# juanaldayparejo/archnemesis-dist

Measured on AMD Instinct MI355X. Metric: forward-models/sec (10k nu x 100 layers), higher is better.
Workload: dtype f64; 1 GPU; synthetic correlated-k nadir thermal-emission forward model: 10000 wavenumbers x 100 layers x 8 gases, G=20, k-table 20Px15T (BASELINE configs[1], SURVEY C2); parallelism=replicas x1 (independent forward models)

## Files before the change

### archnemesis_dist_amd/csrc/ansfm_api.hip

```cpp
#include "ansfm_table_kernels.hip.h"
#include "ansfm_rt_params.h"
#include "ansfm_ctx.hip.h"

using namespace ansfm;

extern "C" {

int ansfm_abi_version(void) { return ANSFM_ABI_VERSION; }

int ansfm_create(int device, ansfm_ctx **out)
{
    if (!out) return ANSFM_ERR_INVALID;
    *out = nullptr;
    int ndev = 0;
    if (hipGetDeviceCount(&ndev) != hipSuccess || ndev <= 0 || device < 0 || device >= ndev)
        return ANSFM_ERR_HIP;
    ansfm_ctx *ctx = new ansfm_ctx();
    ctx->device = device;
    if (hipSetDevice(device) != hipSuccess) { delete ctx; return ANSFM_ERR_HIP; }
    if (hipStreamCreateWithFlags(&ctx->own_stream, hipStreamNonBlocking) != hipSuccess) {
        delete ctx;
        return ANSFM_ERR_HIP;
    }
    ctx->stream = ctx->own_stream;
// ... 95 lines not shown
        hipLaunchKernelGGL(k_table_check, dim3(nblk((size_t)W * Q, 256)), dim3(256), 0, ctx->stream, K_dev, W, G, Q,
                           ctx->d_flag.as<int>());
        hipLaunchKernelGGL(k_table_relayout, dim3((unsigned)(Wpad / kWave), nblk((size_t)Q, 64), (unsigned)G), dim3(256), 0,
                           ctx->stream, K_dev, ctx->lnK.as<double>(), W, Wpad, G, Q);
    }
    HIPCHK(hipGetLastError());
    int flag = 0;
    HIPCHK(hipMemcpyAsync(&flag, ctx->d_flag.p, sizeof(int), hipMemcpyDeviceToHost, ctx->stream));
    HIPCHK(hipStreamSynchronize(ctx->stream));
    ctx->W = W; ctx->Wpad = Wpad; ctx->G = G; ctx->NP = NP; ctx->NT = NT; ctx->S = S;
    ctx->monotone = (flag & 1) ? 0 : 1;
    ctx->has_boxed = (flag & 2) ? 1 : 0;
    ctx->h_delg.assign(DELG, DELG + G);
    ctx->h_wave.assign(WAVE, WAVE + W); ctx->h_press.assign(PRESS, PRESS + NP); ctx->h_temp.assign(TEMP, TEMP + NT);
    ctx->have_table = true;
    ctx->is_lbl = 0; ctx->temp2d = 0;
    ctx->lblrt = 0; ctx->st_n = 0;
    clear_continuum_sources(ctx);
    return build_table_gfast(ctx, Wpad, G, NP * NT * S, false);
}

int ansfm_upload_ktable(ansfm_ctx *ctx, int W, int G, int NP, int NT, int S, const double *K,
                        const double *PRESS, const double *TEMP, const double *WAVE, const double *DELG)
{
    CHECK_CTX(ctx);
    if (W <= 0 || G <= 0 || NP <= 0 || NT <= 0 || S <= 0 || !K) FAIL(ANSFM_ERR_INVALID, "upload_ktable: bad dims");
    HIPCHK(hipSetDevice(ctx->device));
    const size_t n = (size_t)W * G * NP * NT * S;
    HIPCHK(ctx->tmp_in.reserve(n * sizeof(double)));
    HIPCHK(hipMemcpyAsync(ctx->tmp_in.p, K, n * sizeof(double), hipMemcpyHostToDevice, ctx->stream));
// ... 183 lines not shown
        HIPCHK(hipMemcpyAsync(ctx->tmp_in.p, block.data(), block.size() * sizeof(float), hipMemcpyHostToDevice, ctx->stream));
        hipLaunchKernelGGL(k_kta_relayout, dim3(nblk(per_wave * Wpad, 256)), dim3(256), 0, ctx->stream, ctx->tmp_in.as<float>(),
                           ctx->lnK.as<double>(), W, Wpad, G, NP, NT, S, s, ctx->d_flag.as<int>());
        HIPCHK(hipGetLastError());
        HIPCHK(hipStreamSynchronize(ctx->stream));
    }
    int flag = 0;
    HIPCHK(hipMemcpyAsync(&flag, ctx->d_flag.p, sizeof(int), hipMemcpyDeviceToHost, ctx->stream));
    HIPCHK(hipStreamSynchronize(ctx->stream));
    ctx->tmp_in.release();
    ctx->W = W; ctx->Wpad = Wpad; ctx->G = G; ctx->NP = NP; ctx->NT = NT; ctx->S = S;
    ctx->monotone = (flag & 1) ? 0 : 1;
    ctx->has_boxed = (flag & 2) ? 1 : 0;
    ctx->h_delg = DELG; ctx->h_wave = WAVE; ctx->h_press = PRESS; ctx->h_temp = TEMP;
    ctx->have_table = true;
    ctx->is_lbl = lta ? 1 : 0; ctx->temp2d = (lta && hl.temp2d) ? 1 : 0;
    ctx->lblrt = 0; ctx->st_n = 0;
    clear_continuum_sources(ctx);
    if (lta) ctx->monotone = 1;
    ctx->grid_f32 = 1; ctx->delg_f32 = lta ? 0 : 1;
    return build_table_gfast(ctx, Wpad, G, NP * NT * S, lta);
}

int ansfm_upload_ktable_files(ansfm_ctx *ctx, int S, const char *const *paths, double wavemin, double wavemax)
{
    return upload_table_files(ctx, S, paths, wavemin, wavemax, false);
}

int ansfm_upload_lbltable_files(ansfm_ctx *ctx, int S, const char *const *paths, double wavemin, double wavemax)
{
// ... 60 lines not shown
}

int ansfm_last_merge_rowmajor(const ansfm_ctx *cctx, int64_t *merges, int64_t *merges_total)
{
    ansfm_ctx *ctx = const_cast<ansfm_ctx *>(cctx);
    CHECK_CTX(ctx);
    if (!merges || !merges_total) FAIL(ANSFM_ERR_INVALID, "last_merge_rowmajor: null argument");
    *merges = *merges_total = 0;
    if (ctx->d_flag.bytes < kFlagInts * sizeof(int)) return ANSFM_OK;
    HIPCHK(hipSetDevice(ctx->device));
    unsigned long long v[2] = {0, 0};
    HIPCHK(hipMemcpyAsync(v, ctx->d_flag.as<int>() + kFlagTileCounter + 8, sizeof v, hipMemcpyDeviceToHost, ctx->stream));
    HIPCHK(hipStreamSynchronize(ctx->stream));
    *merges = (int64_t)v[0];
    *merges_total = (int64_t)v[1];
    return ANSFM_OK;
}

static void launch_w_to_last(hipStream_t st, unsigned n_batch, const double *src, double *dst, int W, int Wpad, int X1, int X2,
                             int swap12, double padval, size_t src_stride = 0, size_t dst_stride = 0)
{
    const int X = X1 * X2;
    dim3 grid((unsigned)(Wpad / 32), (unsigned)((X + 31) / 32), n_batch);
    hipLaunchKernelGGL(k_transpose_w_last, grid, dim3(32, 8), 0, st, src, dst, W, Wpad, X1, X2, swap12, padval, src_stride,
                       dst_stride);
}

static int read_unsorted(ansfm_ctx *ctx, int *flag)
{
    *flag = 0;
// ... 1099 lines not shown
```

### archnemesis_dist_amd/csrc/ansfm_ctx.hip.h

```cpp
#pragma once
#include <hip/hip_runtime.h>
#include <stdio.h>
#include <stdlib.h>
#include <string.h>

#include <algorithm>
#include <cmath>
#include <initializer_list>
#include <memory>
#include <string>
#include <map>
#include <vector>

#pragma GCC visibility push(default)
#include "../../include/ansfm.h"
#pragma GCC visibility pop
#include "ansfm_merge_plan.h"

namespace ansfm {

struct DevBuf {
    void *p = nullptr;
    size_t bytes = 0;
    DevBuf() = default;
// ... 27 lines not shown

struct FusedRoute {
    DevBuf ws;
    size_t scratch_bytes = 0;
    int recorded = 0;
    hipEvent_t ev[3] = {nullptr, nullptr, nullptr};
    double ms[2] = {0.0, 0.0};
};

}

using ansfm::DevBuf;
using ansfm::FusedRoute;
using ansfm::LblrtIso;

constexpr int kFlagInts = 32, kFlagTileCounter = 16;

struct ansfm_ctx {
    int device = 0;
    hipStream_t own_stream = nullptr;
    hipStream_t stream = nullptr;
    std::string err;
    int num_cus = 256;

    int W = 0, Wpad = 0, G = 0, NP = 0, NT = 0, S = 0;
    int monotone = 0;
    int has_boxed = 1;
    std::vector<double> h_wave, h_press, h_temp;
    DevBuf dcont_gas;
    int dcont_gas_L = 0;
    unsigned grad_gas_mask = 0xFFFFFFFFu;
    std::map<const void *, size_t> merge_lds_allowed;
    ansfm::MergePlan last_merge;
    int merge_keys = 64;
    bool have_table = false;
    int grid_f32 = 0, delg_f32 = 0;
    int is_lbl = 0, temp2d = 0;
    DevBuf lnK, d_press, d_temp, d_wave, d_delg, d_flag;
    DevBuf lnKg;
    size_t lnKg_bytes = 0;
    std::vector<double> h_delg;
    DevBuf cia_tab, cia_idx, cia_lay, dust_kext;
    int cia_on = 0, cia_ispace = 0, cia_NWC = 0, cia_NPAIR = 0, cia_NPE = 0, cia_NT = 0, cia_nfrac = 0, cia_NPARA = 0, cia_NVMR = 0,
        cia_ico2 = -1, cia_in2 = -1, cia_ih2 = -1, cia_covers = 0;
    int dust_n = 0;

    DevBuf li, tau, scratch, cont_t, tmp_in, tmp_out, misc;
    DevBuf dspec_ref, map_out, map_b, map_batch;
    DevBuf dd_slot, dd_work, dd_in;
// ... 156 lines not shown
```

### archnemesis_dist_amd/csrc/ansfm_merge64.hip.h

```cpp
#pragma once
#include <hip/hip_runtime.h>
#include <stdint.h>
#include "ansfm_merge_common.hip.h"

namespace ansfm {

constexpr unsigned kLdsDG = 0, kLdsGORD = kMaxG * 8, kLdsDGF = (2 * kMaxG + 2) * 8, kLdsA = kLdsDGF + kMaxG * 4;


constexpr unsigned kLdsWT = kLdsA;
static_assert(kLdsA == kMergeLdsTables, "the plan's LDS arithmetic");
typedef double dbl2 __attribute__((ext_vector_type(2)));
constexpr unsigned kRecRow = 64u * 16u, kRecBin = 2u * kRecRow;

struct MergeElem {
    double ai, bc, bn, w;
    int ci, np;
};

struct MergeOrient {
    unsigned rbase, cbase;
    unsigned rsh, csh;
    unsigned inc;
};
// ... 249 lines not shown
    }
}
template <int NR>
__device__ __forceinline__ void merge_init(double (&R)[NR], int G, const MergeOrient &mo, double huge)
{
    const double c0 = lds_ld(mo.cbase);
#pragma unroll
    for (int i = 0; i < NR; ++i) {
        const unsigned long long b = (unsigned long long)__double_as_longlong(lds_ld(mo.rbase + (unsigned)(i < G ? i : 0) * 512u) + c0);
        R[i] = (i < G) ? __longlong_as_double((long long)((b & ~0x7FFULL) | (unsigned long long)((unsigned)i << mo.rsh))) : huge;
    }
    merge_init_order<NR>(R, G, huge);
}

template <int NR>
__device__ __forceinline__ bool merge_rowmajor_test(const double (&R)[NR], int G, const MergeOrient &mo)
{
    const double cl = lds_ld(mo.cbase + (unsigned)(G - 1) * 512u);
    const unsigned lowc = (unsigned)(G - 1) << mo.csh;
    bool fail = false;
#pragma unroll
    for (int i = 0; i + 1 < NR; ++i) {
        const unsigned long long b = (unsigned long long)__double_as_longlong(lds_ld(mo.rbase + (unsigned)(i < G ? i : 0) * 512u) + cl);
        const double last = __longlong_as_double((long long)((b & ~0x7FFULL) | (unsigned long long)(((unsigned)i << mo.rsh) | lowc)));
        fail |= (i + 1 < G) & !(last < R[i + 1]);
    }
    return __builtin_amdgcn_ballot_w64(fail) == 0;
}
__host__ __device__ constexpr int merge_rowmajor_sure_cols(int NR)
{
    return NR == 10 ? 9 : NR == 16 ? 11 : NR == 20 ? 17 : NR == 32 ? 21 : 2;
}
template <int NR>
__device__ __forceinline__ void merge_rowmajor_row(double ai, const double (&c)[NR], const double (&w)[NR], int G, WalkState &ws,
                                                   double *rec)
{
#pragma unroll
    for (int j = 0; j < NR; ++j) {
        if (j < merge_rowmajor_sure_cols(NR) || j < G) {
            MergeElem e;
            e.ai = ai; e.bc = c[j]; e.w = w[j];
// ... 64 lines not shown
```

### archnemesis_dist_amd/csrc/ansfm_merge_common.hip.h

```cpp
#pragma once
#include <hip/hip_runtime.h>
#include <stdint.h>
#include "ansfm_merge_plan.h"

namespace ansfm {

__device__ __forceinline__ double encode_lnk(double k)
{
    if (k > 0.0) return log(k);
    unsigned long long b = (unsigned long long)__double_as_longlong(k);
    unsigned long long box = 0x7FF8000000000000ULL | (b >> 13);
    return __longlong_as_double((long long)box);
}
__device__ __forceinline__ bool lnk_is_boxed(double x) { return x != x; }
__device__ __forceinline__ double lnk_unbox(double x)
{
    unsigned long long b = (unsigned long long)__double_as_longlong(x);
    return __longlong_as_double((long long)((b & 0x0007FFFFFFFFFFFFULL) << 13));
}

struct LayerInterp {
    int ipl, iph, itl, ith;
    double v, u, dudt;
};
// ... 45 lines not shown

struct OverlapParams {
    const double *lnK;
    const double *kin;
    const LayerInterp *li;
    const double *amount;
    const double *del_g;
    double *tau;
    double *scratch;
    int *err_flag;
    unsigned int *tile_counter;
    int W, Wpad, G, NT, S, L, n_models;
    int delg_f32;
    double g_ord[kMaxG + 2];
    const double *lnKg;
};
__host__ __device__ constexpr int gfast_stride(int G) { return (G + 1) & ~1; }
typedef double lnk_pair __attribute__((ext_vector_type(2)));


constexpr int kLoadBatch = 10;

template <bool FROM_K, bool NONNEG = false, bool NOBOX = false>
__device__ __forceinline__ void load_gas(const OverlapParams &p, const LayerInterp &q, int m, int l,
                                         int s, int nu, double *DST, int lane, bool &unsorted)
{
    const int G = p.G;
    const double amt = p.amount[((size_t)m * p.S + s) * p.L + l];
    double prev = NONNEG ? 0.0 : -__builtin_inf();
    if constexpr (FROM_K) {
// ... 95 lines not shown
    {0, 0, 100, 2, 0, 0}, {1, 36, 100, 2, 0, 50}, {99, 63, 100, 2, 63, 99}, {50, 17, 100, 2, 33, 8},
    {1, 36, 33, 1, 3, 1}, {32, 63, 33, 1, 63, 32}, {16, 17, 33, 1, 31, 18}, {1, 36, 3, 2, 32, 2}, {2, 63, 3, 2, 63, 2}, {1, 17, 3, 2, 27, 1}};
__host__ __device__ constexpr bool lane_spots_hold()
{
    for (const auto &t : kLaneTileSpots)
        if ((t[2] != 1u && t[2] != (unsigned)kLaneNV) || lane_tile_of(t[0], t[1], t[2] == 1u ? 0u : kLaneNVShift) != t[3]) return false;
    for (const auto &t : kLaneCellSpots) {
        if (t[3] != 1u && t[3] != (unsigned)kLaneNV) return false;
        const LaneCell x = lane_cell(t[0] * 64u + t[1], t[2], t[3] == 1u ? 0u : kLaneNVShift);
        if (x.w != t[4] || x.row != t[5]) return false;
    }
    return true;
}
static_assert(lane_spots_hold(), "lane_tile_of / lane_cell against the model's values");

struct LaneRow {
    int nu;
    unsigned row;
    unsigned arow, krow;
    size_t o1, o2, o3, o4;
    double v, u;
};
template <bool FROM_K>
__device__ __forceinline__ LaneRow lane_row(const OverlapParams &p, int vt, unsigned k, int lane, unsigned nvs, bool gfast)
{
    const unsigned R = (unsigned)p.n_models * (unsigned)p.L;
    const LaneCell cell = lane_cell(k * kWave + (unsigned)lane, R, nvs);
    LaneRow lr;
    lr.row = cell.row;
    lr.nu = vt * kWave + (int)cell.w;
    const unsigned m = lr.row / (unsigned)p.L;
    lr.krow = lr.row - m * (unsigned)p.L;
    lr.arow = m * (unsigned)p.S * (unsigned)p.L + lr.krow;
    lr.o1 = lr.o2 = lr.o3 = lr.o4 = 0;
    lr.v = lr.u = 0.0;
    if constexpr (!FROM_K) {
        const LayerInterp q = p.li[lr.row];
        const size_t strideT = (size_t)p.S * (gfast ? gfast_stride(p.G) : p.G) * p.Wpad;
        const size_t own = gfast ? (size_t)lr.nu * gfast_stride(p.G) : (size_t)lr.nu;
        lr.o1 = ((size_t)q.ipl * p.NT + q.itl) * strideT + own;
        lr.o2 = ((size_t)q.ipl * p.NT + q.ith) * strideT + own;
        lr.o3 = ((size_t)q.iph * p.NT + q.itl) * strideT + own;
        lr.o4 = ((size_t)q.iph * p.NT + q.ith) * strideT + own;
        lr.v = q.v; lr.u = q.u;
    }
// ... 153 lines not shown
```

### archnemesis_dist_amd/csrc/ansfm_merge_plan.h

```cpp
#pragma once
#include <stddef.h>
#include <stdlib.h>
#include <string.h>

#include <type_traits>

#if defined(__HIPCC__)
#define ANSFM_HD __host__ __device__
#else
#define ANSFM_HD
#endif

namespace ansfm {

constexpr int kWave = 64;
constexpr int kMaxG = 32;

constexpr int kOptTable = 1, kOptBfi = 2, kOptExit = 8, kOptOrient = 16;
constexpr int kMergeOpt = kOptTable | kOptBfi | kOptExit | kOptOrient;
constexpr int kOptLaneRows = 32;
constexpr int kOptRowMajor = 64;
constexpr int kFlagLaneRows = 1, kFlagRowMajor = 2;
constexpr int kFlagTableGfast = 4;
ANSFM_HD constexpr bool merge_opt_valid(int opt) { return opt == 0 || (opt & ~kOptTable) == (kOptBfi | kOptExit | kOptOrient); }
ANSFM_HD constexpr int merge_wave_rows(int G, int opt) { return 2 * G + ((opt & kOptOrient) != 0 ? 2 : 1); }
constexpr int kMaxBlockWaves = 8;
ANSFM_HD constexpr unsigned weight_table_bytes(int G) { return (unsigned)(G + 1) * 32u * 8u; }
constexpr int kLaneNV = 2;

constexpr size_t kCuLdsBytes = (size_t)160 * 1024;
constexpr size_t kLdsGranule = 128;
constexpr size_t kMergeLdsTables = (size_t)(2 * kMaxG + 2) * sizeof(double) + kMaxG * sizeof(float);

inline int merge_list_len(int G)
{
    static const int sizes[] = {8, 10, 16, 20, 32};
    for (int v : sizes) if (v >= G) return v;
    return 32;
}
template <class F>
auto by_list_len(int G, F &&f)
{
    switch (merge_list_len(G)) {
        case 8: return f(std::integral_constant<int, 8>{});
        case 10: return f(std::integral_constant<int, 10>{});
        case 16: return f(std::integral_constant<int, 16>{});
        case 20: return f(std::integral_constant<int, 20>{});
        default: return f(std::integral_constant<int, 32>{});
    }
}

inline long merge_grid(int num_cus, size_t block_bytes, int max_per_cu, long ntiles)
{
    int per_cu = (int)(kCuLdsBytes / block_bytes);
// ... 2 lines not shown
    long grid = (long)num_cus * per_cu;
    if (grid > ntiles) grid = ntiles;
    return grid < 1 ? 1 : grid;
}

struct MergeSwitches {
    enum Lanes { kLanesUnset, kLanesWavenumbers, kLanesPairs };
    bool walk_records = false;
    bool load_boxtests = false;
    bool legacy = false;
    int keys = 0;
    int waves_per_cu = 0;
    Lanes lanes = kLanesUnset;
    bool rowmajor_off = false;
    bool layout_wave = false;
};
inline MergeSwitches merge_switches_from_env()
{
    MergeSwitches sw;
    const auto is = [](const char *name, const char *value) { const char *ev = getenv(name); return ev && !strcmp(ev, value); };
    const auto starts = [](const char *name, char c) { const char *ev = getenv(name); return ev && ev[0] == c; };
    sw.walk_records = is("ANSFM_MERGE_WALK", "records");
    sw.load_boxtests = starts("ANSFM_LOAD_BOXTESTS", '1');
    sw.legacy = starts("ANSFM_MERGE_LEGACY", '1');
    if (const char *ev = getenv("ANSFM_MERGE_KEYS")) sw.keys = atoi(ev) == 32 ? 32 : 64;
    if (const char *ev = getenv("ANSFM_WAVES_PER_CU")) sw.waves_per_cu = atoi(ev);
    if (is("ANSFM_MERGE_LANES", "wavenumbers")) sw.lanes = MergeSwitches::kLanesWavenumbers;
    else if (is("ANSFM_MERGE_LANES", "pairs")) sw.lanes = MergeSwitches::kLanesPairs;
    sw.rowmajor_off = starts("ANSFM_MERGE_ROWMAJOR", '0');
    sw.layout_wave = is("ANSFM_TABLE_LAYOUT", "wave");
    return sw;
}

struct MergeCall {
    bool from_k = false;
    bool generic = false;
    bool monotone = false;
    bool has_boxed = true;
    bool delg_f32 = false;
    int merge_keys = 64;
    int G = 0, S = 0, W = 0, Wpad = 0, L = 0, n_models = 0, num_cus = 0;
    double w00 = 0.0, g_ord1 = 0.0;
    bool gfast_copy = false;
    int table_W = 0, table_Wpad = 0, table_G = 0, table_S = 0;
    size_t lds32 = 0;
};

struct MergePlan {
    bool sorted = false, nodiv = false, nobox = false, keys32 = false;
    int opt = 0;
    bool lane_rows = false, rowmajor = false, gfast = false;
    int lane_nv = 0, flags = 0;
    int nwaves = 1;
    size_t lds = 0;
    long grid = 1;
    size_t scratch_bytes_per_block = 0;
    int trims = 0, group_width = 0;
};

inline MergePlan merge_plan(const MergeCall &c, const MergeSwitches &sw)
{
    MergePlan m;
    m.sorted = !c.generic && (c.from_k || c.monotone);
    m.nodiv = m.sorted && c.G >= 2 && c.w00 < c.g_ord1 && !sw.walk_records;
    m.nobox = m.nodiv && !c.from_k && !c.has_boxed && !sw.load_boxtests;
    m.keys32 = m.nodiv && (sw.keys != 0 ? sw.keys : c.merge_keys) == 32;
    const bool trimmed = m.nodiv && !sw.legacy && !m.keys32;
// ... 10 lines not shown
        m.lds = shared_bytes + (size_t)m.nwaves * wave_bytes;
        const long per_cu = merge_grid(c.num_cus, m.lds, 1, ntiles), needed = (ntiles + m.nwaves - 1) / m.nwaves;
        m.grid = per_cu < needed ? per_cu : needed;
    } else {
        m.nwaves = 1;
        m.lds = m.keys32 ? c.lds32 : wave_bytes + kMergeLdsTables + (m.sorted ? 0 : (size_t)2 * c.G * kWave);
        m.grid = merge_grid(c.num_cus, (m.lds + kLdsGranule - 1) / kLdsGranule * kLdsGranule, max_per_cu, ntiles);
    }
    m.scratch_bytes_per_block = (size_t)m.nwaves * 6 * c.G * kWave * sizeof(double);

    m.lane_rows = m.opt != 0 && (long)c.n_models * c.L < (1L << 24) && sw.lanes != MergeSwitches::kLanesWavenumbers;
    m.lane_nv = m.opt == 0 ? 0 : sw.lanes == MergeSwitches::kLanesPairs ? kLaneNV : 1;
    m.rowmajor = table && !sw.rowmajor_off;
    m.gfast = m.lane_rows && !c.from_k && c.gfast_copy && c.W == c.table_W && c.Wpad == c.table_Wpad && c.G == c.table_G &&
              c.S == c.table_S && !sw.layout_wave;
    m.flags = (m.lane_rows ? kFlagLaneRows : 0) | (m.rowmajor ? kFlagRowMajor : 0) | (m.gfast ? kFlagTableGfast : 0);
    m.trims = m.opt | (m.lane_rows ? kOptLaneRows : 0) | (m.rowmajor ? kOptRowMajor : 0);
    m.group_width = m.lane_rows ? m.lane_nv : 0;
    return m;
}

}
```

### archnemesis_dist_amd/csrc/ansfm_overlap.hip

```cpp
#include "ansfm_overlap_kernels.hip.h"
#include "ansfm_merge32_launch.h"
#include "ansfm_ctx.hip.h"

namespace ansfm {

void merge_params(ansfm_ctx *ctx, OverlapParams &p, const double *kin, int W, int Wpad, int G, int S, int L, int n_models,
                  const LayerInterp *li, const double *amount, const double *del_g_dev, const double *del_g_host, double *tau)
{
    p.lnK = ctx->lnK.as<double>();
    p.kin = kin;
    p.li = li;
    p.amount = amount;
    p.del_g = del_g_dev;
    p.tau = tau;
    p.err_flag = ctx->d_flag.as<int>() + 1;
    p.tile_counter = reinterpret_cast<unsigned int *>(ctx->d_flag.as<int>() + kFlagTileCounter);
    p.W = W; p.Wpad = Wpad; p.G = G; p.NT = ctx->NT; p.S = S; p.L = L; p.n_models = n_models;
    p.delg_f32 = ctx->delg_f32;
    double acc = 0.0;
    float accf = 0.0f;
    p.g_ord[0] = 0.0;
    for (int g = 0; g < G; ++g) {
        if (ctx->delg_f32) { accf += (float)del_g_host[g]; p.g_ord[g + 1] = (double)accf; }
        else { acc += del_g_host[g]; p.g_ord[g + 1] = acc; }
    }
    p.g_ord[G] = 1.0;
    p.g_ord[G + 1] = __builtin_nan("");
}

int merge_launch_begin(ansfm_ctx *ctx, const OverlapParams &p, long grid, std::initializer_list<MergeWorkspace> workspaces)
{
    for (const MergeWorkspace &w : workspaces) HIPCHK(w.buf->reserve((size_t)grid * w.bytes_per_block));
    HIPCHK(hipMemsetAsync(p.tile_counter, 0, (8 + 4) * sizeof(unsigned int), ctx->stream));
    return ANSFM_OK;
}

using MergeKernel = void (*)(OverlapParams, int, int);

template <int D, bool FK, bool W32>
static MergeKernel overlap_kernel_of(const MergePlan &m)
{
    constexpr int kTrimmed = W32 ? kMergeOpt : (kMergeOpt & ~kOptTable);
    if (m.opt == kTrimmed) return m.nobox ? k_ck_overlap<D, false, W32, true, true, true, kTrimmed> : k_ck_overlap<D, FK, W32, true, true, false, kTrimmed>;
    if (m.opt != 0) return nullptr;
    if (m.nodiv) return m.nobox ? k_ck_overlap<D, false, W32, true, true, true> : k_ck_overlap<D, FK, W32, true, true>;
    return m.sorted ? k_ck_overlap<D, FK, W32, true> : k_ck_overlap<D, FK, W32, false>;
}

// ... 23 lines not shown
    c.from_k = from_k; c.generic = generic; c.monotone = ctx->monotone != 0; c.has_boxed = ctx->has_boxed != 0; c.delg_f32 = w32;
    c.merge_keys = ctx->merge_keys;
    c.G = G; c.S = S; c.W = W; c.Wpad = Wpad; c.L = L; c.n_models = n_models; c.num_cus = ctx->num_cus;
    c.w00 = w32 ? (double)((float)del_g_host[0] * (float)del_g_host[0]) : del_g_host[0] * del_g_host[0];
    c.g_ord1 = p.g_ord[1];
    c.gfast_copy = ctx->lnKg_bytes != 0 && !ctx->is_lbl;
    c.table_W = ctx->W; c.table_Wpad = ctx->Wpad; c.table_G = ctx->G; c.table_S = ctx->S;
    c.lds32 = overlap32_lds_bytes(G, w32);
    const MergePlan m = merge_plan(c, merge_switches_from_env());

    const int rc = merge_launch_begin(ctx, p, m.grid, {{&ctx->scratch, m.scratch_bytes_per_block}});
    if (rc) return rc;
    p.scratch = ctx->scratch.as<double>();
    if (m.gfast) p.lnKg = ctx->lnKg.as<double>();
    ctx->last_merge = m;
    if (m.keys32) {
        HIPCHK(launch_overlap32(p, from_k, (unsigned)m.grid, ctx->stream));
        return ANSFM_OK;
    }
    const MergeKernel kern = overlap_kernel(m, from_k, w32, G);
    if (!kern) FAIL(ANSFM_ERR_UNSUPPORTED, "forward merge: no kernel is compiled for this plan");
    if (m.lds > (size_t)64 * 1024) {
        size_t &lds_allowed = ctx->merge_lds_allowed[reinterpret_cast<const void *>(kern)];
        if (m.lds > lds_allowed) {
            HIPCHK(hipFuncSetAttribute(reinterpret_cast<const void *>(kern), hipFuncAttributeMaxDynamicSharedMemorySize, (int)m.lds));
            lds_allowed = m.lds;
        }
    }
    hipLaunchKernelGGL(kern, dim3((unsigned)m.grid), dim3(kWave * m.nwaves), m.lds, ctx->stream, p, m.flags, m.lane_nv);
    HIPCHK(hipGetLastError());
    return ANSFM_OK;
}

}
```

### archnemesis_dist_amd/csrc/ansfm_overlap_kernels.hip.h

```cpp
#pragma once
#include "ansfm_merge64.hip.h"

namespace ansfm {


template <bool FROM_K, bool NOBOX, int OPT>
__device__ __forceinline__ void load_cell(const OverlapParams &p, int lane_rows, bool gfast, const LaneRow &lr, const LayerInterp &q, int m,
                                          int l, int s, int nu, double *DST, int lane, bool &unsorted)
{
    if constexpr (OPT != 0) {
        if (lane_rows != 0) {
            if (!FROM_K && gfast) load_gas_rows<FROM_K, NOBOX, true>(p, lr, s, DST, lane, unsorted);
            else load_gas_rows<FROM_K, NOBOX, false>(p, lr, s, DST, lane, unsorted);
            return;
        }
    }
    load_gas<FROM_K, false, NOBOX>(p, q, m, l, s, nu, DST, lane, unsorted);
}

template <int NR, bool FROM_K, bool W32, bool SORTED = true, bool NODIV = false, bool NOBOX = false, int OPT = 0>
__global__ __launch_bounds__((OPT & kOptTable) != 0 ? kWave * kMaxBlockWaves : kWave) __attribute__((amdgpu_waves_per_eu(1, 2)))
void k_ck_overlap(OverlapParams p, int flags, int lane_nv)
{
    static_assert(OPT == 0 || (SORTED && NODIV), "the fast path");
    static_assert(merge_opt_valid(OPT), "OPT == 0 || (OPT & ~kOptTable) == (kOptBfi | kOptExit | kOptOrient)");
    constexpr bool kTable = (OPT & kOptTable) != 0, kOrient = (OPT & kOptOrient) != 0;
    static_assert(!kTable || W32, "the weight table holds float32 products only (launch_overlap)");
    const int lane_rows = kTable ? (flags & kFlagLaneRows) : flags;
    const bool gfast = !FROM_K && OPT != 0 && (flags & kFlagTableGfast) != 0;
    const unsigned nvs = lane_nv == 1 ? 0u : kLaneNVShift;
    unsigned n_rowmajor = 0, n_merged = 0;
    extern __shared__ double smem[];
    const int lane = kTable ? (int)(threadIdx.x & 63u) : (int)threadIdx.x;
    const int wv = kTable ? __builtin_amdgcn_readfirstlane((int)(threadIdx.x >> 6)) : 0;
    const int nwv = kTable ? (int)(blockDim.x >> 6) : 1;
    const int G = p.G;
    double *DG = smem;
    double *GORD = DG + kMaxG;
    double *A = reinterpret_cast<double *>(reinterpret_cast<char *>(GORD + kMaxG + 2) + kMaxG * sizeof(float));
    if constexpr (kTable) {
        double *WT = A;
        for (int idx = (int)threadIdx.x; idx < (G + 1) * 32; idx += (int)blockDim.x) {
            const int row = idx & 31, col = idx >> 5;
            double w = 0.0;
            if (row < G && col < G) w = (double)((float)p.del_g[row] * (float)p.del_g[col]);
            WT[idx] = w;
// ... 14 lines not shown
    __syncthreads();
    double wsum = 0.0;
    for (int g = 0; g < G; ++g) wsum += DG[g];
    const double wtot = wsum * wsum;

    double *rec = p.scratch + ((size_t)blockIdx.x * nwv + wv) * 6 * G * kWave;
    TileQueue tq;
    tq.init();
    for (;;) {
        int vt = 0, m = 0, l = 0;
        LaneRow lr{};
        if constexpr (OPT != 0) {
            if (lane_rows != 0) {
                unsigned k = 0;
                if (!tq.next_rows(p, lane, nvs, vt, k)) break;
                lr = lane_row<FROM_K>(p, vt, k, lane, nvs, gfast);
            } else if (!tq.next(p, lane, vt, m, l)) break;
        } else {
            if (!tq.next(p, lane, vt, m, l)) break;
        }
        const int nu = vt * kWave + lane;
        LayerInterp q;
        if constexpr (!FROM_K) q = p.li[(size_t)m * p.L + l];
        bool unsorted = false;

        load_cell<FROM_K, NOBOX, OPT>(p, lane_rows, gfast, lr, q, m, l, 0, nu, A, lane, unsorted);
        double alast = A[(G - 1) * kWave + lane];
        if constexpr (!SORTED) sort_column(A, PA, G, lane);
        for (int s = 1; s < p.S; ++s) {
            load_cell<FROM_K, NOBOX, OPT>(p, lane_rows, gfast, lr, q, m, l, s, nu, B, lane, unsorted);
            if constexpr (SORTED)
                if (__builtin_amdgcn_ballot_w64(unsorted) != 0) break;
            const double blast = B[(G - 1) * kWave + lane];
            if constexpr (!SORTED) sort_column(B, PB, G, lane);
            if constexpr (SORTED) alast = A[(G - 1) * kWave + lane];
            bool takeB, keepA;
            if (s == 1) { takeB = (alast <= 0.0); keepA = !takeB && (blast <= 0.0); }
            else { keepA = (blast <= 0.0); takeB = !keepA && (alast <= 0.0); }
            const bool do_merge = !(takeB | keepA);
// ... 13 lines not shown
                    if (__builtin_amdgcn_ballot_w64(swapped) != 0) {
                        double prev = A[lane];
                        for (int g = 1; g < G; ++g) {
                            const double v = A[g * kWave + lane];
                            swapped &= (v >= prev);
                            prev = v;
                        }
                    }
                    mo = merge_orient(lds_addr(A + lane), lds_addr(B + lane), swapped);
                    merge_init<NR>(R, G, mo, HUGE_KEY);
                } else
                    merge_init<NR>(R, G, lane, A, B[lane], HUGE_KEY);
                MergeElem e0, e1;
                WalkState ws;
                if constexpr (kTable) {
                    if ((flags & kFlagRowMajor) != 0 && merge_rowmajor_test<NR>(R, G, mo)) {
                        ws = walk_begin(GORD, lane);
                        merge_rowmajor<NR>(G, mo, ws, rec);
                        walked = true;
                    }
                }
                if (!kTable || !walked) {
                merge_fetch<W32, SORTED, OPT>(R[0], lane, A, B, DG, e0, PA, PB, mo);
                ws = walk_begin(GORD, lane);
                const int nloop = G * G - (G - 1);
                constexpr int kPer = 2;
                for (int n = nloop / kPer; n > 0; --n) {
                    merge_step<NR, W32, false, SORTED, NODIV, NR, OPT>(R, e0, e1, ws, lane, A, B, DG, GORD, rec, PA, PB, mo);
                    merge_step<NR, W32, false, SORTED, NODIV, NR, OPT>(R, e1, e0, ws, lane, A, B, DG, GORD, rec, PA, PB, mo);
                }
                merge_step<NR, W32, false, SORTED, NODIV, NR, OPT>(R, e0, e1, ws, lane, A, B, DG, GORD, rec, PA, PB, mo);
                if (((G ^ NR) & 1) != 0) { const MergeElem t = e0; e0 = e1; e1 = t; }
                merge_peel<NR - 1, NR, W32, SORTED, NODIV, OPT>(R, e0, e1, ws, G, lane, A, B, DG, GORD, rec, PA, PB, mo);
                }
                if constexpr (NODIV) {
// ... 70 lines not shown
                if constexpr (!SORTED) {
                    for (int g = 0; g < G; ++g) PA[g * kWave + lane] = (unsigned char)g;
                    alast = A[(G - 1) * kWave + lane];
                }
            }
            if constexpr (kTable) {
                n_merged += __builtin_amdgcn_ballot_w64(do_merge) != 0 ? 1u : 0u;
                n_rowmajor += __builtin_amdgcn_ballot_w64(walked) != 0 ? 1u : 0u;
            }
        }
        if constexpr (OPT != 0) {
            if (lane_rows != 0) {
                if (unsorted) atomicOr(p.err_flag, 1);
                double *outr = p.tau + ((size_t)lr.row * G) * p.Wpad + lr.nu;
                for (int g = 0; g < G; ++g) outr[(size_t)g * p.Wpad] = A[g * kWave + lane];
                continue;
            }
        }
        double *out = p.tau + (((size_t)m * p.L + l) * G) * p.Wpad + nu;
        if constexpr (SORTED) {
            if (unsorted) atomicOr(p.err_flag, 1);
            for (int g = 0; g < G; ++g) out[(size_t)g * p.Wpad] = A[g * kWave + lane];
        } else {
            for (int g = 0; g < G; ++g) out[(size_t)PA[g * kWave + lane] * p.Wpad] = A[g * kWave + lane];
        }
    }
    if constexpr (kTable) {
        unsigned long long *cnt = reinterpret_cast<unsigned long long *>(p.tile_counter + 8);
        if (lane == 0) {
            atomicAdd(cnt, (unsigned long long)n_rowmajor);
            atomicAdd(cnt + 1, (unsigned long long)n_merged);
        }
    }
}

}
```

### archnemesis_dist_amd/engine.py

```python
import contextlib
import ctypes as C
import os
import numpy as np

from . import _lib

_f8 = np.float64


def _np(a, dtype=_f8):
    return None if a is None else np.ascontiguousarray(a, dtype=dtype)


def _is_f32(a):
    return getattr(a, "dtype", None) == np.float32


def _ptr(a):
    if a is None:
        return None
    if isinstance(a, np.ndarray):
        return a.ctypes.data_as(C.c_void_p)
    return C.c_void_p(a.data_ptr())

# ... 222 lines not shown

    def ktable_gfast(self):
        p, b = C.c_int(), C.c_int64()
        self._check(self._lib.ansfm_ktable_gfast(self._ctx, C.byref(p), C.byref(b)), "ktable_gfast")
        return bool(p.value), int(b.value)

    def last_merge_table_layout(self):
        g = C.c_int()
        self._check(self._lib.ansfm_last_merge_table_layout(self._ctx, C.byref(g)), "last_merge_table_layout")
        return bool(g.value)

    def last_merge_rowmajor(self):
        m, t = C.c_int64(), C.c_int64()
        self._check(self._lib.ansfm_last_merge_rowmajor(self._ctx, C.byref(m), C.byref(t)), "last_merge_rowmajor")
        return int(m.value), int(t.value)

    def calc_k(self, press, temp, grad=False):
        press = _np(press); temp = _np(temp)
        W, G, NP, NT, S = self.dims
        L = press.shape[0]
        k = np.empty((W, G, L, S)); dk = np.empty((W, G, L, S)) if grad else None
        self._check(self._lib.ansfm_calc_k(self._ctx, L, _ptr(press), _ptr(temp), _ptr(k), _ptr(dk)), "calc_k")
        return (k, dk) if grad else k

    def k_overlap(self, del_g, k_w_g_l_gas, amount_layer):
        self.set_f32_semantics(getattr(self, "grid_f32", False), _is_f32(del_g))
        del_g = _np(del_g); k = _np(k_w_g_l_gas); am = _np(amount_layer)
        W, G, L, S = k.shape
        if am.shape != (S, L):
            raise ValueError("amount_layer must be (NGAS, NLAYER)")
# ... 1226 lines not shown
```

### include/ansfm.h

```cpp
#ifndef ANSFM_H
#define ANSFM_H

#include <stdint.h>

#ifdef __cplusplus
extern "C" {
#endif

#define ANSFM_ABI_VERSION 1

#define ANSFM_OK 0
#define ANSFM_ERR_INVALID 1
#define ANSFM_ERR_HIP 2
#define ANSFM_ERR_NOTABLE 3
#define ANSFM_ERR_UNSORTED 4
#define ANSFM_ERR_UNSUPPORTED 5

#define ANSFM_MAX_NG 32
#define ANSFM_MAX_CONT_GRAD_SLOTS 48

typedef struct ansfm_ctx ansfm_ctx;

int ansfm_abi_version(void);

// ... 7 lines not shown
int ansfm_set_f32_semantics(ansfm_ctx *ctx, int grid_f32, int delg_f32);

int ansfm_upload_ktable(ansfm_ctx *ctx, int W, int G, int NP, int NT, int S, const double *K,
                        const double *PRESS, const double *TEMP, const double *WAVE,
                        const double *DELG);
int ansfm_upload_ktable_dev(ansfm_ctx *ctx, int W, int G, int NP, int NT, int S,
                            const double *K_dev, const double *PRESS, const double *TEMP,
                            const double *WAVE, const double *DELG);
int ansfm_ktable_info(const ansfm_ctx *ctx, int64_t dims[5], int *monotone);
int ansfm_ktable_has_boxed(const ansfm_ctx *ctx, int *has_boxed);
int ansfm_last_merge_launch(const ansfm_ctx *ctx, int *waves_per_block, int *trims);
int ansfm_last_merge_rowmajor(const ansfm_ctx *ctx, int64_t *merges, int64_t *merges_total);
int ansfm_last_merge_group_width(const ansfm_ctx *ctx, int *width);
int ansfm_ktable_gfast(const ansfm_ctx *ctx, int *present, int64_t *bytes);
int ansfm_last_merge_table_layout(const ansfm_ctx *ctx, int *gfast);

int ansfm_upload_lbltable(ansfm_ctx *ctx, int W, int NP, int NT, int S, const double *K,
                          const double *PRESS, const double *TEMP, int temp2d, const double *WAVE);
int ansfm_calc_klbl(ansfm_ctx *ctx, int L, const double *press, const double *temp, double *k_out,
                    double *dkdT_out);

int ansfm_ktable_file_header(const char *path, int64_t dims[4], int32_t ids[2], double hdr[3], double *wave,
                             float *g_ord, float *del_g, float *press, float *temp);
int ansfm_upload_ktable_files(ansfm_ctx *ctx, int S, const char *const *paths, double wavemin, double wavemax);
int ansfm_ktable_grids(const ansfm_ctx *ctx, double *WAVE, double *PRESS, double *TEMP, double *DELG);
int ansfm_lbltable_file_header(const char *path, int64_t dims[3], int32_t ids[2], double hdr[2], double *wave,
                               float *press, float *temp);
int ansfm_upload_lbltable_files(ansfm_ctx *ctx, int S, const char *const *paths, double wavemin, double wavemax);

int ansfm_kdist_bins(ansfm_ctx *ctx, int ncalc, const double *wavecalc, const double *kabs, int nbin,
// ... 350 lines not shown
```

Measured before the change: 280.5 forward-models/s.

## Reorder wavenumber lanes by per-gas fast-merge hint recorded on the previous call

The merge kernel now records, for one representative row, a byte per wavenumber giving which gases passed the row-major fast-merge test. On the next call with the same table and shape it ranks the lanes of each wavefront by that byte, using readlane and ds_permute, so wavenumbers with the same pass pattern share a wavefront. The aim is to cut divergence where the ballot-based fast path fails for the whole wave because of a few lanes. It adds per-tile rank computation, a double-buffered hint buffer keyed by table generation, and a dependence on behaviour carried across calls.

```diff
diff --git a/archnemesis_dist_amd/csrc/ansfm_api.hip b/archnemesis_dist_amd/csrc/ansfm_api.hip
--- a/archnemesis_dist_amd/csrc/ansfm_api.hip
+++ b/archnemesis_dist_amd/csrc/ansfm_api.hip
@@ -133,6 +133,7 @@
     ctx->h_delg.assign(DELG, DELG + G);
     ctx->h_wave.assign(WAVE, WAVE + W); ctx->h_press.assign(PRESS, PRESS + NP); ctx->h_temp.assign(TEMP, TEMP + NT);
     ctx->have_table = true;
+    ++ctx->table_generation;
     ctx->is_lbl = 0; ctx->temp2d = 0;
     ctx->lblrt = 0; ctx->st_n = 0;
     clear_continuum_sources(ctx);
@@ -346,6 +347,7 @@
     ctx->has_boxed = (flag & 2) ? 1 : 0;
     ctx->h_delg = DELG; ctx->h_wave = WAVE; ctx->h_press = PRESS; ctx->h_temp = TEMP;
     ctx->have_table = true;
+    ++ctx->table_generation;
     ctx->is_lbl = lta ? 1 : 0; ctx->temp2d = (lta && hl.temp2d) ? 1 : 0;
     ctx->lblrt = 0; ctx->st_n = 0;
     clear_continuum_sources(ctx);
@@ -436,6 +438,22 @@
     HIPCHK(hipStreamSynchronize(ctx->stream));
     *merges = (int64_t)v[0];
     *merges_total = (int64_t)v[1];
+    return ANSFM_OK;
+}
+
+int ansfm_last_merge_order(const ansfm_ctx *cctx, int *applied, int64_t *valid_bytes_nonzero)
+{
+    ansfm_ctx *ctx = const_cast<ansfm_ctx *>(cctx);
+    CHECK_CTX(ctx);
+    if (!applied || !valid_bytes_nonzero) FAIL(ANSFM_ERR_INVALID, "last_merge_order: null argument");
+    *applied = ctx->last_merge_ordered ? 1 : 0;
+    *valid_bytes_nonzero = 0;
+    if (!ctx->last_merge_ordered || ctx->d_flag.bytes < kFlagInts * sizeof(int)) return ANSFM_OK;
+    HIPCHK(hipSetDevice(ctx->device));
+    unsigned long long v = 0;
+    HIPCHK(hipMemcpyAsync(&v, ctx->d_flag.as<int>() + kFlagTileCounter + 8 + 4, sizeof v, hipMemcpyDeviceToHost, ctx->stream));
+    HIPCHK(hipStreamSynchronize(ctx->stream));
+    *valid_bytes_nonzero = (int64_t)v;
     return ANSFM_OK;
 }
 
diff --git a/archnemesis_dist_amd/csrc/ansfm_ctx.hip.h b/archnemesis_dist_amd/csrc/ansfm_ctx.hip.h
--- a/archnemesis_dist_amd/csrc/ansfm_ctx.hip.h
+++ b/archnemesis_dist_amd/csrc/ansfm_ctx.hip.h
@@ -65,7 +65,8 @@
 using ansfm::FusedRoute;
 using ansfm::LblrtIso;
 
-constexpr int kFlagInts = 32, kFlagTileCounter = 16;
+constexpr int kFlagInts = 32, kFlagTileCounter = 16, kMergeTotals = 3;
+static_assert(kFlagTileCounter + 8 + 2 * kMergeTotals <= kFlagInts, "the totals lie inside d_flag");
 
 struct ansfm_ctx {
     int device = 0;
@@ -84,6 +85,18 @@
     std::map<const void *, size_t> merge_lds_allowed;
     ansfm::MergePlan last_merge;
     int merge_keys = 64;
+    DevBuf merge_hint;
+    int merge_hint_parity = 0;
+    struct MergeHintKey {
+        long source = -1;
+        int W = 0, Wpad = 0, R = 0, S = 0, G = 0;
+        bool operator==(const MergeHintKey &o) const
+        {
+            return source == o.source && W == o.W && Wpad == o.Wpad && R == o.R && S == o.S && G == o.G;
+        }
+    } merge_hint_key;
+    long table_generation = 0;
+    bool last_merge_ordered = false;
     bool have_table = false;
     int grid_f32 = 0, delg_f32 = 0;
     int is_lbl = 0, temp2d = 0;
diff --git a/archnemesis_dist_amd/csrc/ansfm_merge64.hip.h b/archnemesis_dist_amd/csrc/ansfm_merge64.hip.h
--- a/archnemesis_dist_amd/csrc/ansfm_merge64.hip.h
+++ b/archnemesis_dist_amd/csrc/ansfm_merge64.hip.h
@@ -287,7 +287,7 @@
 }
 
 template <int NR>
-__device__ __forceinline__ bool merge_rowmajor_test(const double (&R)[NR], int G, const MergeOrient &mo)
+__device__ __forceinline__ bool merge_rowmajor_test(const double (&R)[NR], int G, const MergeOrient &mo, bool &lane_passes)
 {
     const double cl = lds_ld(mo.cbase + (unsigned)(G - 1) * 512u);
     const unsigned lowc = (unsigned)(G - 1) << mo.csh;
@@ -298,6 +298,7 @@
         const double last = __longlong_as_double((long long)((b & ~0x7FFULL) | (unsigned long long)(((unsigned)i << mo.rsh) | lowc)));
         fail |= (i + 1 < G) & !(last < R[i + 1]);
     }
+    lane_passes = !fail;
     return __builtin_amdgcn_ballot_w64(fail) == 0;
 }
 __host__ __device__ constexpr int merge_rowmajor_sure_cols(int NR)
diff --git a/archnemesis_dist_amd/csrc/ansfm_merge_common.hip.h b/archnemesis_dist_amd/csrc/ansfm_merge_common.hip.h
--- a/archnemesis_dist_amd/csrc/ansfm_merge_common.hip.h
+++ b/archnemesis_dist_amd/csrc/ansfm_merge_common.hip.h
@@ -83,6 +83,8 @@
     int delg_f32;
     double g_ord[kMaxG + 2];
     const double *lnKg;
+    const unsigned char *hint_in;
+    unsigned char *hint_out;
 };
 __host__ __device__ constexpr int gfast_stride(int G) { return (G + 1) & ~1; }
 typedef double lnk_pair __attribute__((ext_vector_type(2)));
@@ -208,6 +210,42 @@
 }
 static_assert(lane_spots_hold(), "lane_tile_of / lane_cell against the model's values");
 
+__host__ __device__ constexpr unsigned merge_order_key(unsigned byte, unsigned i) { return (byte << 6) | i; }
+template <class F>
+__host__ __device__ constexpr unsigned merge_order_rank(F &&b, unsigned i)
+{
+    unsigned r = 0;
+    for (unsigned j = 0; j < 64u; ++j) r += merge_order_key(b(j), j) < merge_order_key(b(i), i) ? 1u : 0u;
+    return r;
+}
+constexpr unsigned kOrderSpotReal = 58, kOrderSpotMul = 37, kOrderSpotAdd = 11, kOrderSpotMask = 0xE0;
+__host__ __device__ constexpr unsigned merge_order_spot_byte(unsigned i)
+{
+    return i < kOrderSpotReal ? (i * kOrderSpotMul + kOrderSpotAdd) & kOrderSpotMask : 0xFFu;
+}
+constexpr unsigned kOrderSpots[][2] = {{0, 0}, {1, 7}, {2, 15}, {3, 22}, {6, 50}, {7, 1}, {13, 51}, {31, 31}, {57, 21}, {58, 58}, {63, 63}};
+__host__ __device__ constexpr bool order_spots_hold()
+{
+    for (const auto &t : kOrderSpots)
+        if (merge_order_rank([](unsigned i) { return merge_order_spot_byte(i); }, t[0]) != t[1]) return false;
+    for (unsigned i = 0; i < 64u; ++i)
+        if (merge_order_rank([](unsigned) { return 0u; }, i) != i) return false;
+    return true;
+}
+static_assert(order_spots_hold(), "merge_order_rank against the model's values");
+
+__device__ __forceinline__ int merge_order_inverse(const unsigned char *hint_in, int vt, int W, int lane, bool &nonzero)
+{
+    const int nu = vt * kWave + lane;
+    const unsigned byte = nu < W ? (unsigned)hint_in[nu] : 0xFFu;
+    nonzero = nu < W && byte != 0u;
+    const unsigned key = merge_order_key(byte, (unsigned)lane);
+    unsigned rank = 0;
+#pragma unroll
+    for (int j = 0; j < kWave; ++j) rank += (unsigned)__builtin_amdgcn_readlane((int)key, j) < key ? 1u : 0u;
+    return __builtin_amdgcn_ds_permute((int)(rank << 2), lane);
+}
+
 struct LaneRow {
     int nu;
     unsigned row;
@@ -216,13 +254,14 @@
     double v, u;
 };
 template <bool FROM_K>
-__device__ __forceinline__ LaneRow lane_row(const OverlapParams &p, int vt, unsigned k, int lane, unsigned nvs, bool gfast)
+__device__ __forceinline__ LaneRow lane_row(const OverlapParams &p, int vt, unsigned k, int lane, unsigned nvs, bool gfast,
+                                            bool ordered = false, int inv = 0)
 {
     const unsigned R = (unsigned)p.n_models * (unsigned)p.L;
     const LaneCell cell = lane_cell(k * kWave + (unsigned)lane, R, nvs);
     LaneRow lr;
     lr.row = cell.row;
-    lr.nu = vt * kWave + (int)cell.w;
+    lr.nu = vt * kWave + (ordered ? __builtin_amdgcn_ds_bpermute((int)(cell.w << 2), inv) : (int)cell.w);
     const unsigned m = lr.row / (unsigned)p.L;
     lr.krow = lr.row - m * (unsigned)p.L;
     lr.arow = m * (unsigned)p.S * (unsigned)p.L + lr.krow;
diff --git a/archnemesis_dist_amd/csrc/ansfm_merge_plan.h b/archnemesis_dist_amd/csrc/ansfm_merge_plan.h
--- a/archnemesis_dist_amd/csrc/ansfm_merge_plan.h
+++ b/archnemesis_dist_amd/csrc/ansfm_merge_plan.h
@@ -38,6 +38,7 @@
     for (int v : sizes) if (v >= G) return v;
     return 32;
 }
+constexpr int kMergeOrderMinList = 16;
 template <class F>
 auto by_list_len(int G, F &&f)
 {
@@ -70,6 +71,7 @@
     Lanes lanes = kLanesUnset;
     bool rowmajor_off = false;
     bool layout_wave = false;
+    bool order_off = false;
 };
 inline MergeSwitches merge_switches_from_env()
 {
@@ -85,6 +87,7 @@
     else if (is("ANSFM_MERGE_LANES", "pairs")) sw.lanes = MergeSwitches::kLanesPairs;
     sw.rowmajor_off = starts("ANSFM_MERGE_ROWMAJOR", '0');
     sw.layout_wave = is("ANSFM_TABLE_LAYOUT", "wave");
+    sw.order_off = starts("ANSFM_MERGE_ORDER", '0');
     return sw;
 }
 
@@ -107,6 +110,7 @@
     int opt = 0;
     bool lane_rows = false, rowmajor = false, gfast = false;
     int lane_nv = 0, flags = 0;
+    bool order = false;
     int nwaves = 1;
     size_t lds = 0;
     long grid = 1;
@@ -147,6 +151,7 @@
     m.rowmajor = table && !sw.rowmajor_off;
     m.gfast = m.lane_rows && !c.from_k && c.gfast_copy && c.W == c.table_W && c.Wpad == c.table_Wpad && c.G == c.table_G &&
               c.S == c.table_S && !sw.layout_wave;
+    m.order = m.rowmajor && m.lane_rows && m.lane_nv == 1 && merge_list_len(c.G) >= kMergeOrderMinList && !sw.order_off;
     m.flags = (m.lane_rows ? kFlagLaneRows : 0) | (m.rowmajor ? kFlagRowMajor : 0) | (m.gfast ? kFlagTableGfast : 0);
     m.trims = m.opt | (m.lane_rows ? kOptLaneRows : 0) | (m.rowmajor ? kOptRowMajor : 0);
     m.group_width = m.lane_rows ? m.lane_nv : 0;
diff --git a/archnemesis_dist_amd/csrc/ansfm_overlap.hip b/archnemesis_dist_amd/csrc/ansfm_overlap.hip
--- a/archnemesis_dist_amd/csrc/ansfm_overlap.hip
+++ b/archnemesis_dist_amd/csrc/ansfm_overlap.hip
@@ -31,7 +31,7 @@
 int merge_launch_begin(ansfm_ctx *ctx, const OverlapParams &p, long grid, std::initializer_list<MergeWorkspace> workspaces)
 {
     for (const MergeWorkspace &w : workspaces) HIPCHK(w.buf->reserve((size_t)grid * w.bytes_per_block));
-    HIPCHK(hipMemsetAsync(p.tile_counter, 0, (8 + 4) * sizeof(unsigned int), ctx->stream));
+    HIPCHK(hipMemsetAsync(p.tile_counter, 0, (8 + 2 * kMergeTotals) * sizeof(unsigned int), ctx->stream));
     return ANSFM_OK;
 }
 
@@ -85,6 +85,18 @@
     p.scratch = ctx->scratch.as<double>();
     if (m.gfast) p.lnKg = ctx->lnKg.as<double>();
     ctx->last_merge = m;
+    ctx->last_merge_ordered = false;
+    ansfm_ctx::MergeHintKey key;
+    bool valid = false;
+    if (m.order) {
+        key.source = from_k ? 0 : ctx->table_generation;
+        key.W = W; key.Wpad = Wpad; key.R = n_models * L; key.S = S; key.G = G;
+        HIPCHK(ctx->merge_hint.reserve((size_t)2 * Wpad));
+        valid = key == ctx->merge_hint_key;
+        if (!valid) HIPCHK(hipMemsetAsync(ctx->merge_hint.p, 0, (size_t)2 * Wpad, ctx->stream));
+        p.hint_in = ctx->merge_hint.as<unsigned char>() + (size_t)ctx->merge_hint_parity * Wpad;
+        p.hint_out = ctx->merge_hint.as<unsigned char>() + (size_t)(1 - ctx->merge_hint_parity) * Wpad;
+    }
     if (m.keys32) {
         HIPCHK(launch_overlap32(p, from_k, (unsigned)m.grid, ctx->stream));
         return ANSFM_OK;
@@ -100,6 +112,11 @@
     }
     hipLaunchKernelGGL(kern, dim3((unsigned)m.grid), dim3(kWave * m.nwaves), m.lds, ctx->stream, p, m.flags, m.lane_nv);
     HIPCHK(hipGetLastError());
+    if (m.order) {
+        ctx->merge_hint_parity ^= 1;
+        ctx->merge_hint_key = key;
+        ctx->last_merge_ordered = valid;
+    }
     return ANSFM_OK;
 }
 
diff --git a/archnemesis_dist_amd/csrc/ansfm_overlap_kernels.hip.h b/archnemesis_dist_amd/csrc/ansfm_overlap_kernels.hip.h
--- a/archnemesis_dist_amd/csrc/ansfm_overlap_kernels.hip.h
+++ b/archnemesis_dist_amd/csrc/ansfm_overlap_kernels.hip.h
@@ -30,6 +30,8 @@
     const bool gfast = !FROM_K && OPT != 0 && (flags & kFlagTableGfast) != 0;
     const unsigned nvs = lane_nv == 1 ? 0u : kLaneNVShift;
     unsigned n_rowmajor = 0, n_merged = 0;
+    const bool ordered = kTable && p.hint_in != nullptr;
+    unsigned n_hints = 0;
     extern __shared__ double smem[];
     const int lane = kTable ? (int)(threadIdx.x & 63u) : (int)threadIdx.x;
     const int wv = kTable ? __builtin_amdgcn_readfirstlane((int)(threadIdx.x >> 6)) : 0;
@@ -74,6 +76,15 @@
             if (lane_rows != 0) {
                 unsigned k = 0;
                 if (!tq.next_rows(p, lane, nvs, vt, k)) break;
+                if constexpr (kTable) {
+                    int inv = lane;
+                    if (ordered) {
+                        bool nonzero = false;
+                        inv = merge_order_inverse(p.hint_in, vt, p.W, lane, nonzero);
+                        if (k == 0) n_hints += (unsigned)__builtin_popcountll(__builtin_amdgcn_ballot_w64(nonzero));
+                    }
+                    lr = lane_row<FROM_K>(p, vt, k, lane, nvs, gfast, ordered, inv);
+                } else
                 lr = lane_row<FROM_K>(p, vt, k, lane, nvs, gfast);
             } else if (!tq.next(p, lane, vt, m, l)) break;
         } else {
@@ -83,6 +94,7 @@
         LayerInterp q;
         if constexpr (!FROM_K) q = p.li[(size_t)m * p.L + l];
         bool unsorted = false;
+        unsigned pattern = 0;
 
         load_cell<FROM_K, NOBOX, OPT>(p, lane_rows, gfast, lr, q, m, l, 0, nu, A, lane, unsorted);
         double alast = A[(G - 1) * kWave + lane];
@@ -126,11 +138,13 @@
                 MergeElem e0, e1;
                 WalkState ws;
                 if constexpr (kTable) {
-                    if ((flags & kFlagRowMajor) != 0 && merge_rowmajor_test<NR>(R, G, mo)) {
+                    bool lane_passes = false;
+                    if ((flags & kFlagRowMajor) != 0 && merge_rowmajor_test<NR>(R, G, mo, lane_passes)) {
                         ws = walk_begin(GORD, lane);
                         merge_rowmajor<NR>(G, mo, ws, rec);
                         walked = true;
                     }
+                    pattern |= lane_passes && s <= 8 ? 0x100u >> s : 0u;
                 }
                 if (!kTable || !walked) {
                 merge_fetch<W32, SORTED, OPT>(R[0], lane, A, B, DG, e0, PA, PB, mo);
@@ -231,6 +245,10 @@
                 if (unsorted) atomicOr(p.err_flag, 1);
                 double *outr = p.tau + ((size_t)lr.row * G) * p.Wpad + lr.nu;
                 for (int g = 0; g < G; ++g) outr[(size_t)g * p.Wpad] = A[g * kWave + lane];
+                if constexpr (kTable) {
+                    if (ordered && lr.row == (((unsigned)p.n_models * (unsigned)p.L) >> 1) && lr.nu < p.W)
+                        p.hint_out[lr.nu] = (unsigned char)pattern;
+                }
                 continue;
             }
         }
@@ -247,6 +265,7 @@
         if (lane == 0) {
             atomicAdd(cnt, (unsigned long long)n_rowmajor);
             atomicAdd(cnt + 1, (unsigned long long)n_merged);
+            if (ordered) atomicAdd(cnt + 2, (unsigned long long)n_hints);
         }
     }
 }
diff --git a/archnemesis_dist_amd/engine.py b/archnemesis_dist_amd/engine.py
--- a/archnemesis_dist_amd/engine.py
+++ b/archnemesis_dist_amd/engine.py
@@ -260,6 +260,11 @@
         m, t = C.c_int64(), C.c_int64()
         self._check(self._lib.ansfm_last_merge_rowmajor(self._ctx, C.byref(m), C.byref(t)), "last_merge_rowmajor")
         return int(m.value), int(t.value)
+
+    def last_merge_order(self):
+        a, n = C.c_int(), C.c_int64()
+        self._check(self._lib.ansfm_last_merge_order(self._ctx, C.byref(a), C.byref(n)), "last_merge_order")
+        return bool(a.value), int(n.value)
 
     def calc_k(self, press, temp, grad=False):
         press = _np(press); temp = _np(temp)
diff --git a/include/ansfm.h b/include/ansfm.h
--- a/include/ansfm.h
+++ b/include/ansfm.h
@@ -45,6 +45,7 @@
 int ansfm_last_merge_group_width(const ansfm_ctx *ctx, int *width);
 int ansfm_ktable_gfast(const ansfm_ctx *ctx, int *present, int64_t *bytes);
 int ansfm_last_merge_table_layout(const ansfm_ctx *ctx, int *gfast);
+int ansfm_last_merge_order(const ansfm_ctx *ctx, int *applied, int64_t *valid_bytes_nonzero);
 
 int ansfm_upload_lbltable(ansfm_ctx *ctx, int W, int NP, int NT, int S, const double *K,
                           const double *PRESS, const double *TEMP, int temp2d, const double *WAVE);
```

Measured after the change: 288.0 forward-models/s (median of 6 runs). +2.7%, better.
